# dbolya/yolact

Measured on AMD Instinct MI355X. Metric: images/sec (550x550, batch 8 per GPU), YOLACT yolact_resnet50 forward + Detect (Fast NMS), higher is better.
Workload: dtype f32 (fp32 in / fp32 accumulate / fp32 out; 92 % of the GEMM time on fp16x2 tiles = every fp32 operand as two fp16 pieces by round to nearest (22 significant bits + 2 signs: exact for ~2/3 of all fp32 values, one fp32 ulp otherwise), 3 exact piece products per product on the fp16 matrix pipe; measure

## Files before the change

yolact_amd/csrc/stem.hip:

```cpp
#include "common.h"
#include <stdlib.h>
#include "../../include/yolact_amd.h"

int ymi_internal_prof_begin(double flops, int tile, int kind, hipStream_t s);
void ymi_internal_prof_end(int idx, hipStream_t s);

namespace {

typedef _Float16 f16x8 __attribute__((ext_vector_type(8)));
typedef _Float16 f16x4 __attribute__((ext_vector_type(4)));

constexpr int NTHR = 512, NWAVE = 8;
constexpr int PH = 4, PW = 6;
constexpr int SH = 2 * PH + 1, SW = 2 * PW + 1;
constexpr int IH = 2 * SH + 5, IW = 2 * SW + 5;
constexpr int IPITCH = 32;
constexpr int NPATCH = IH * IPITCH;
constexpr int KPAD = 224, KSTEPS = KPAD / 16;
constexpr int WPITCH = KPAD * 2 + 16;
constexpr int COUT = 64;
constexpr int EPITCH = COUT + 1;

struct StemParams {
  const float *x; float *y;
  int B, H, W, Hs, Ws, Hp, Wp, tiles_x, tiles_y, ntiles;
  const unsigned short *w;
  int cout_pad;
  const float *scale, *bias;
  float *y_amax;
};

__device__ __forceinline__ int crow(int r, int lane) { return (r & 3) + 8 * (r >> 2) + 4 * (lane >> 5); }

__global__ __launch_bounds__(NTHR) void stem_pool_k(const StemParams p) {
#if defined(__HIP_DEVICE_COMPILE__)
  constexpr int WB = 0, WPLANE = COUT * WPITCH;
  constexpr int PB = 2 * WPLANE, PPLANE = NPATCH * 8;
  constexpr int EB = PB + 2 * PPLANE;
  constexpr int RED = EB + 128 * EPITCH * 4;
  constexpr int LDS_BYTES = RED + 64;
  static_assert(LDS_BYTES <= 160 * 1024, "LDS");
  __shared__ __attribute__((aligned(16))) unsigned char lds[LDS_BYTES];

  const int t = threadIdx.x, lane = t & 63, wave = __builtin_amdgcn_readfirstlane(t >> 6);
  const int hh = lane >> 5;
  const ymi_amax_pre apre = ymi_amax_prefetch(p.y_amax);

  for (int u = t; u < 2 * COUT * (KPAD / 8); u += NTHR) {
    const int plane = u / (COUT * (KPAD / 8)), r = u - plane * (COUT * (KPAD / 8));
    const int row = r / (KPAD / 8), g8 = r - row * (KPAD / 8);
    const f16x8 v = *reinterpret_cast<const f16x8 *>(p.w + ((size_t)plane * p.cout_pad + row) * KPAD + 8 * g8);
    *reinterpret_cast<f16x8 *>(lds + WB + plane * WPLANE + row * WPITCH + g8 * 16) = v;
  }
  const int mt = wave & 3, nt = wave >> 2;
  const int ncol = nt * 32 + (lane & 31);
  const float sc = p.scale[ncol], bi = p.bias[ncol];
  const int m = mt * 32 + (lane & 31);
  const int mi = m < SH * SW ? m / SW : 0, mj = m < SH * SW ? m - (m / SW) * SW : 0;
  const int abase = ((2 * mi) * IPITCH + 2 * mj) * 8;
  float *red = reinterpret_cast<float *>(lds + RED);
  float *et = reinterpret_cast<float *>(lds + EB);

  auto fetch = [&](int tile, float (&v)[2][3]) {
    const int b = tile / (p.tiles_x * p.tiles_y), tt = tile - b * (p.tiles_x * p.tiles_y);
    const int ty = tt / p.tiles_x, tx = tt - ty * p.tiles_x;
    const int iy0 = 4 * (ty * PH) - 5, ix0 = 4 * (tx * PW) - 5;
#pragma unroll
    for (int k = 0; k < 2; ++k) {
      const int slot = t + NTHR * k, r = slot >> 5, c = slot & 31;
      const int iy = iy0 + r, ix = ix0 + c;
      const bool ok = slot < NPATCH && c < IW && (unsigned)iy < (unsigned)p.H && (unsigned)ix < (unsigned)p.W;
      const float *src = p.x + ((size_t)b * 3 * p.H + (ok ? iy : 0)) * p.W + (ok ? ix : 0);
#pragma unroll
      for (int ch = 0; ch < 3; ++ch) v[k][ch] = ok ? src[(size_t)ch * p.H * p.W] : 0.f;
    }
  };
  float cur[2][3], nxt[2][3];
  int tile = blockIdx.x;
  if (tile < p.ntiles) fetch(tile, cur);
  float amy = 0.f;
  __syncthreads();
  for (; tile < p.ntiles; tile += gridDim.x) {
    const int b = tile / (p.tiles_x * p.tiles_y), tt = tile - b * (p.tiles_x * p.tiles_y);
    const int ty = tt / p.tiles_x, tx = tt - ty * p.tiles_x;
    float am = 0.f;
#pragma unroll
    for (int k = 0; k < 2; ++k)
#pragma unroll
      for (int ch = 0; ch < 3; ++ch) am = fmaxf(am, fabsf(cur[k][ch]));
    {
      const unsigned mx = ymi_wave_umax63(__float_as_uint(am));
      if (lane == 63) red[wave] = __uint_as_float(mx);
    }
    __syncthreads();
    float pm = 0.f;
#pragma unroll
    for (int w = 0; w < NWAVE; ++w) pm = fmaxf(pm, red[w]);
    float s, inv;
    ymi_h2_scale(pm, s, inv);
#pragma unroll
    for (int k = 0; k < 2; ++k) {
      const int slot = t + NTHR * k;
      if (slot < NPATCH) {
        f16x4 h, l;
#pragma unroll
        for (int ch = 0; ch < 3; ++ch) {
          const float tv = cur[k][ch] * s;
          h[ch] = (_Float16)tv;
          l[ch] = (_Float16)(tv - (float)h[ch]);
        }
        h[3] = (_Float16)0.f; l[3] = (_Float16)0.f;
        *reinterpret_cast<f16x4 *>(lds + PB + slot * 8) = h;
        *reinterpret_cast<f16x4 *>(lds + PB + PPLANE + slot * 8) = l;
      }
    }
    const int next = tile + gridDim.x;
    if (next < p.ntiles) fetch(next, nxt);
    __syncthreads();
    f32x16 acc;
#pragma unroll
    for (int r = 0; r < 16; ++r) acc[r] = 0.f;
    const unsigned char *wrow = lds + WB + ncol * WPITCH;
#pragma unroll
    for (int ks = 0; ks < KSTEPS; ++ks) {
      constexpr int NT = 49;
      const int ta0 = 4 * ks < NT ? 4 * ks : NT - 1, ta1 = 4 * ks + 1 < NT ? 4 * ks + 1 : NT - 1;
      const int tb0 = 4 * ks + 2 < NT ? 4 * ks + 2 : NT - 1, tb1 = 4 * ks + 3 < NT ? 4 * ks + 3 : NT - 1;
      const int oa0 = ((ta0 / 7) * IPITCH + ta0 % 7) * 8, oa1 = ((ta1 / 7) * IPITCH + ta1 % 7) * 8;
      const int ob0 = ((tb0 / 7) * IPITCH + tb0 % 7) * 8, ob1 = ((tb1 / 7) * IPITCH + tb1 % 7) * 8;
      const int o0 = abase + (hh ? ob0 : oa0), o1 = abase + (hh ? ob1 : oa1);
      const f16x4 h0 = *reinterpret_cast<const f16x4 *>(lds + PB + o0), h1 = *reinterpret_cast<const f16x4 *>(lds + PB + o1);
      const f16x4 l0 = *reinterpret_cast<const f16x4 *>(lds + PB + PPLANE + o0), l1 = *reinterpret_cast<const f16x4 *>(lds + PB + PPLANE + o1);
      const f16x8 ah = {h0[0], h0[1], h0[2], h0[3], h1[0], h1[1], h1[2], h1[3]};
      const f16x8 al = {l0[0], l0[1], l0[2], l0[3], l1[0], l1[1], l1[2], l1[3]};
      const f16x8 bh = *reinterpret_cast<const f16x8 *>(wrow + (16 * ks + 8 * hh) * 2);
      const f16x8 bl = *reinterpret_cast<const f16x8 *>(wrow + WPLANE + (16 * ks + 8 * hh) * 2);
      acc = ymi_mfma32(ah, bl, acc);
      acc = ymi_mfma32(al, bh, acc);
      acc = ymi_mfma32(ah, bh, acc);
    }
    const int sy0 = 2 * (ty * PH) - 1, sx0 = 2 * (tx * PW) - 1;
#pragma unroll
    for (int r = 0; r < 16; ++r) {
      const int row = mt * 32 + crow(r, lane);
      const int i = row / SW, j = row - i * SW;
      const bool ok = row < SH * SW && (unsigned)(sy0 + i) < (unsigned)p.Hs && (unsigned)(sx0 + j) < (unsigned)p.Ws;
      float v = (acc[r] * inv) * sc + bi;
      v = v > 0.f ? v : 0.f;
      et[row * EPITCH + ncol] = ok ? v : -__builtin_inff();
    }
    __syncthreads();
    const int c = t & 63;
#pragma unroll
    for (int k = 0; k < (PH * PW + 7) / 8; ++k) {
      const int q = (t >> 6) + 8 * k;
      if (q < PH * PW) {
        const int qy = q / PW, qx = q - qy * PW;
        const int py = ty * PH + qy, px = tx * PW + qx;
        float mx = -__builtin_inff();
#pragma unroll
        for (int dy = 0; dy < 3; ++dy)
#pragma unroll
          for (int dx = 0; dx < 3; ++dx) mx = fmaxf(mx, et[((2 * qy + dy) * SW + 2 * qx + dx) * EPITCH + c]);
        if (py < p.Hp && px < p.Wp) {
          p.y[(((size_t)b * p.Hp + py) * p.Wp + px) * COUT + c] = mx;
          amy = fmaxf(amy, fabsf(mx));
        }
      }
    }
#pragma unroll
    for (int k = 0; k < 2; ++k)
#pragma unroll
      for (int ch = 0; ch < 3; ++ch) cur[k][ch] = nxt[k][ch];
  }
  if (p.y_amax) ymi_amax_finish(apre, amy);
#endif
}

}

extern "C" int ymi_stem_pool_f32(const ymi_stem_desc *d, void *stream) {
  if (!d) return YMI_ENULL;
  if (!d->x || !d->y || !d->w_h2 || !d->scale_h2 || !d->bias) return YMI_ENULL;
  if (d->B <= 0 || d->H < 7 || d->W < 7) return YMI_EARG;
  if (d->cout_pad < COUT || d->kpad != KPAD) return YMI_ESHAPE;
  if ((((uintptr_t)d->w_h2) | ((uintptr_t)d->y)) & 15) return YMI_ESHAPE;
  StemParams p;
  p.x = d->x; p.y = d->y; p.B = d->B; p.H = d->H; p.W = d->W;
  p.Hs = (d->H + 6 - 7) / 2 + 1; p.Ws = (d->W + 6 - 7) / 2 + 1;
  p.Hp = (p.Hs + 2 - 3) / 2 + 1; p.Wp = (p.Ws + 2 - 3) / 2 + 1;
  if ((long)d->B * 3 * d->H * d->W >= (1L << 31) || (long)d->B * p.Hp * p.Wp * COUT >= (1L << 31)) return YMI_ESHAPE;
  p.tiles_x = (p.Wp + PW - 1) / PW; p.tiles_y = (p.Hp + PH - 1) / PH;
  p.ntiles = p.tiles_x * p.tiles_y * d->B;
  p.w = (const unsigned short *)d->w_h2; p.cout_pad = d->cout_pad;
  p.scale = d->scale_h2; p.bias = d->bias; p.y_amax = d->y_amax;
  hipStream_t s = (hipStream_t)stream;
  const double flops = 2.0 * d->B * p.Hs * p.Ws * 64.0 * 147.0;
  const int pr = ymi_internal_prof_begin(flops, YMI_TILE_H2 | YMI_TILE_64x64, 8, s);
  int dev = 0, cus = 256;
  hipGetDevice(&dev);
  hipDeviceGetAttribute(&cus, hipDeviceAttributeMultiprocessorCount, dev);
  const int grid = p.ntiles < cus ? p.ntiles : cus;
  hipLaunchKernelGGL(stem_pool_k, dim3(grid), dim3(NTHR), 0, s, p);
  const int rc = ymi_launch_status();
  ymi_internal_prof_end(pr, s);
  return rc;
}
```

Measured before the change: 2346.

## Restructure stem conv+pool kernel: smaller tiles, register weights, 2 WGs per CU

Shrinks the stem tile (3x4 pooled outputs, 64 M rows) and the workgroup to 256 threads so two workgroups fit per CU. The grid grows to twice the CU count. Weights move from LDS into registers, and the patch goes into a 4-phase parity layout to cut LDS bank conflicts. Interior tiles skip per-row bounds checks, and the pooling pass uses float4 loads and stores. The next-tile prefetch now overwrites the current register buffer, and optional timing stamps are gated behind YMI_DIAGNOSTICS. Smaller tiles increase halo redundancy and register pressure from keeping all weights resident.

```diff
diff --git a/yolact_amd/csrc/stem.hip b/yolact_amd/csrc/stem.hip
--- a/yolact_amd/csrc/stem.hip
+++ b/yolact_amd/csrc/stem.hip
@@ -10,16 +10,21 @@
 typedef _Float16 f16x8 __attribute__((ext_vector_type(8)));
 typedef _Float16 f16x4 __attribute__((ext_vector_type(4)));
 
-constexpr int NTHR = 512, NWAVE = 8;
-constexpr int PH = 4, PW = 6;
+constexpr int NTHR = 256, NWAVE = 4, WG_PER_CU = 2;
+constexpr int PH = 3, PW = 4;
 constexpr int SH = 2 * PH + 1, SW = 2 * PW + 1;
+constexpr int MROWS = 64;
 constexpr int IH = 2 * SH + 5, IW = 2 * SW + 5;
-constexpr int IPITCH = 32;
-constexpr int NPATCH = IH * IPITCH;
+constexpr int IPITCH = 24;
+constexpr int NFETCH = IH * IPITCH;
+constexpr int NF = (NFETCH + NTHR - 1) / NTHR;
+static_assert(SH * SW <= MROWS && IW <= IPITCH, "tile");
+constexpr int PPITCH = 41, PROWS = 11, PPLANE = PROWS * PPITCH;
+constexpr int NPSLOT = 4 * PPLANE;
+static_assert(PPITCH % 32 == SW % 32 && PPITCH >= (IW + 1) / 2 && PROWS >= (MROWS - 1) / SW + 4 && (NPSLOT * 8) % 16 == 0, "patch image");
 constexpr int KPAD = 224, KSTEPS = KPAD / 16;
-constexpr int WPITCH = KPAD * 2 + 16;
 constexpr int COUT = 64;
-constexpr int EPITCH = COUT + 1;
+constexpr int EPITCH = COUT;
 
 struct StemParams {
   const float *x; float *y;
@@ -28,80 +33,102 @@
   int cout_pad;
   const float *scale, *bias;
   float *y_amax;
+  unsigned long long *trace;
 };
 
+#ifdef YMI_DIAGNOSTICS
+#define STEM_STAMP(i) { const unsigned long long n_ = __builtin_amdgcn_s_memtime(); tr_[i] += n_ - last_; last_ = n_; }
+#else
+#define STEM_STAMP(i)
+#endif
+
+
 __device__ __forceinline__ int crow(int r, int lane) { return (r & 3) + 8 * (r >> 2) + 4 * (lane >> 5); }
-
-__global__ __launch_bounds__(NTHR) void stem_pool_k(const StemParams p) {
+__host__ __device__ constexpr int pslot(int r, int c) { return ((r & 1) * 2 + (c & 1)) * PPLANE + (r >> 1) * PPITCH + (c >> 1); }
+
+__global__ __launch_bounds__(NTHR, 2) void stem_pool_k(const StemParams p) {
 #if defined(__HIP_DEVICE_COMPILE__)
-  constexpr int WB = 0, WPLANE = COUT * WPITCH;
-  constexpr int PB = 2 * WPLANE, PPLANE = NPATCH * 8;
-  constexpr int EB = PB + 2 * PPLANE;
-  constexpr int RED = EB + 128 * EPITCH * 4;
-  constexpr int LDS_BYTES = RED + 64;
-  static_assert(LDS_BYTES <= 160 * 1024, "LDS");
+  constexpr int PB = 0, PL = NPSLOT * 8;
+  constexpr int EB = PB + 2 * PL;
+  constexpr int RED = EB + MROWS * EPITCH * 4;
+  constexpr int PIX = RED + 64;
+  constexpr int HALF = PIX + MROWS * 4;
+  constexpr int LDS_BYTES = HALF + NTHR * 4;
+  static_assert(WG_PER_CU * LDS_BYTES <= 160 * 1024, "LDS");
   __shared__ __attribute__((aligned(16))) unsigned char lds[LDS_BYTES];
 
   const int t = threadIdx.x, lane = t & 63, wave = __builtin_amdgcn_readfirstlane(t >> 6);
   const int hh = lane >> 5;
   const ymi_amax_pre apre = ymi_amax_prefetch(p.y_amax);
-
-  for (int u = t; u < 2 * COUT * (KPAD / 8); u += NTHR) {
-    const int plane = u / (COUT * (KPAD / 8)), r = u - plane * (COUT * (KPAD / 8));
-    const int row = r / (KPAD / 8), g8 = r - row * (KPAD / 8);
-    const f16x8 v = *reinterpret_cast<const f16x8 *>(p.w + ((size_t)plane * p.cout_pad + row) * KPAD + 8 * g8);
-    *reinterpret_cast<f16x8 *>(lds + WB + plane * WPLANE + row * WPITCH + g8 * 16) = v;
+#ifdef YMI_DIAGNOSTICS
+  unsigned long long tr_[8] = {0, 0, 0, 0, 0, 0, 0, 0}, last_ = __builtin_amdgcn_s_memtime();
+#endif
+
+  const int mw = wave & 1, nt = wave >> 1;
+  const int ncol = nt * 32 + (lane & 31);
+  f16x8 bh[KSTEPS], bl[KSTEPS];
+  {
+    const unsigned short *wr = p.w + (size_t)ncol * KPAD + 8 * hh;
+    const size_t plane = (size_t)p.cout_pad * KPAD;
+#pragma unroll
+    for (int ks = 0; ks < KSTEPS; ++ks) {
+      bh[ks] = *reinterpret_cast<const f16x8 *>(wr + 16 * ks);
+      bl[ks] = *reinterpret_cast<const f16x8 *>(wr + plane + 16 * ks);
+    }
   }
-  const int mt = wave & 3, nt = wave >> 2;
-  const int ncol = nt * 32 + (lane & 31);
+  for (int u = t; u < 2 * PL / 16; u += NTHR) *reinterpret_cast<f32x4 *>(lds + PB + u * 16) = f32x4{0.f, 0.f, 0.f, 0.f};
   const float sc = p.scale[ncol], bi = p.bias[ncol];
-  const int m = mt * 32 + (lane & 31);
-  const int mi = m < SH * SW ? m / SW : 0, mj = m < SH * SW ? m - (m / SW) * SW : 0;
-  const int abase = ((2 * mi) * IPITCH + 2 * mj) * 8;
+  const int m0 = mw * 32 + (lane & 31);
+  const int abase = ((m0 / SW) * PPITCH + m0 % SW) * 8;
   float *red = reinterpret_cast<float *>(lds + RED);
   float *et = reinterpret_cast<float *>(lds + EB);
-
-  auto fetch = [&](int tile, float (&v)[2][3]) {
+  int *pix = reinterpret_cast<int *>(lds + PIX);
+  if (t < MROWS) pix[t] = ((t / SW) << 8) | (t % SW);
+  reinterpret_cast<int *>(lds + HALF)[t] = hh;
+
+  auto fetch = [&](int tile, float (&v)[NF][3]) {
     const int b = tile / (p.tiles_x * p.tiles_y), tt = tile - b * (p.tiles_x * p.tiles_y);
     const int ty = tt / p.tiles_x, tx = tt - ty * p.tiles_x;
     const int iy0 = 4 * (ty * PH) - 5, ix0 = 4 * (tx * PW) - 5;
 #pragma unroll
-    for (int k = 0; k < 2; ++k) {
-      const int slot = t + NTHR * k, r = slot >> 5, c = slot & 31;
+    for (int k = 0; k < NF; ++k) {
+      const int slot = t + NTHR * k, r = slot / IPITCH, c = slot % IPITCH;
       const int iy = iy0 + r, ix = ix0 + c;
-      const bool ok = slot < NPATCH && c < IW && (unsigned)iy < (unsigned)p.H && (unsigned)ix < (unsigned)p.W;
+      const bool ok = slot < NFETCH && c < IW && (unsigned)iy < (unsigned)p.H && (unsigned)ix < (unsigned)p.W;
       const float *src = p.x + ((size_t)b * 3 * p.H + (ok ? iy : 0)) * p.W + (ok ? ix : 0);
 #pragma unroll
       for (int ch = 0; ch < 3; ++ch) v[k][ch] = ok ? src[(size_t)ch * p.H * p.W] : 0.f;
     }
   };
-  float cur[2][3], nxt[2][3];
+  float cur[NF][3];
   int tile = blockIdx.x;
   if (tile < p.ntiles) fetch(tile, cur);
   float amy = 0.f;
-  __syncthreads();
+  STEM_STAMP(0);
   for (; tile < p.ntiles; tile += gridDim.x) {
     const int b = tile / (p.tiles_x * p.tiles_y), tt = tile - b * (p.tiles_x * p.tiles_y);
     const int ty = tt / p.tiles_x, tx = tt - ty * p.tiles_x;
     float am = 0.f;
 #pragma unroll
-    for (int k = 0; k < 2; ++k)
+    for (int k = 0; k < NF; ++k)
 #pragma unroll
       for (int ch = 0; ch < 3; ++ch) am = fmaxf(am, fabsf(cur[k][ch]));
     {
       const unsigned mx = ymi_wave_umax63(__float_as_uint(am));
       if (lane == 63) red[wave] = __uint_as_float(mx);
     }
+    STEM_STAMP(1);
     __syncthreads();
+    STEM_STAMP(2);
     float pm = 0.f;
 #pragma unroll
     for (int w = 0; w < NWAVE; ++w) pm = fmaxf(pm, red[w]);
     float s, inv;
     ymi_h2_scale(pm, s, inv);
 #pragma unroll
-    for (int k = 0; k < 2; ++k) {
-      const int slot = t + NTHR * k;
-      if (slot < NPATCH) {
+    for (int k = 0; k < NF; ++k) {
+      const int slot = t + NTHR * k, r = slot / IPITCH, c = slot % IPITCH;
+      if (slot < NFETCH && c < IW) {
         f16x4 h, l;
 #pragma unroll
         for (int ch = 0; ch < 3; ++ch) {
@@ -110,70 +137,95 @@
           l[ch] = (_Float16)(tv - (float)h[ch]);
         }
         h[3] = (_Float16)0.f; l[3] = (_Float16)0.f;
-        *reinterpret_cast<f16x4 *>(lds + PB + slot * 8) = h;
-        *reinterpret_cast<f16x4 *>(lds + PB + PPLANE + slot * 8) = l;
+        *reinterpret_cast<f16x4 *>(lds + PB + pslot(r, c) * 8) = h;
+        *reinterpret_cast<f16x4 *>(lds + PB + PL + pslot(r, c) * 8) = l;
       }
     }
     const int next = tile + gridDim.x;
-    if (next < p.ntiles) fetch(next, nxt);
+    if (next < p.ntiles) fetch(next, cur);
+    STEM_STAMP(3);
     __syncthreads();
-    f32x16 acc;
-#pragma unroll
-    for (int r = 0; r < 16; ++r) acc[r] = 0.f;
-    const unsigned char *wrow = lds + WB + ncol * WPITCH;
-#pragma unroll
-    for (int ks = 0; ks < KSTEPS; ++ks) {
-      constexpr int NT = 49;
-      const int ta0 = 4 * ks < NT ? 4 * ks : NT - 1, ta1 = 4 * ks + 1 < NT ? 4 * ks + 1 : NT - 1;
-      const int tb0 = 4 * ks + 2 < NT ? 4 * ks + 2 : NT - 1, tb1 = 4 * ks + 3 < NT ? 4 * ks + 3 : NT - 1;
-      const int oa0 = ((ta0 / 7) * IPITCH + ta0 % 7) * 8, oa1 = ((ta1 / 7) * IPITCH + ta1 % 7) * 8;
-      const int ob0 = ((tb0 / 7) * IPITCH + tb0 % 7) * 8, ob1 = ((tb1 / 7) * IPITCH + tb1 % 7) * 8;
-      const int o0 = abase + (hh ? ob0 : oa0), o1 = abase + (hh ? ob1 : oa1);
-      const f16x4 h0 = *reinterpret_cast<const f16x4 *>(lds + PB + o0), h1 = *reinterpret_cast<const f16x4 *>(lds + PB + o1);
-      const f16x4 l0 = *reinterpret_cast<const f16x4 *>(lds + PB + PPLANE + o0), l1 = *reinterpret_cast<const f16x4 *>(lds + PB + PPLANE + o1);
-      const f16x8 ah = {h0[0], h0[1], h0[2], h0[3], h1[0], h1[1], h1[2], h1[3]};
-      const f16x8 al = {l0[0], l0[1], l0[2], l0[3], l1[0], l1[1], l1[2], l1[3]};
-      const f16x8 bh = *reinterpret_cast<const f16x8 *>(wrow + (16 * ks + 8 * hh) * 2);
-      const f16x8 bl = *reinterpret_cast<const f16x8 *>(wrow + WPLANE + (16 * ks + 8 * hh) * 2);
-      acc = ymi_mfma32(ah, bl, acc);
-      acc = ymi_mfma32(al, bh, acc);
-      acc = ymi_mfma32(ah, bh, acc);
-    }
+    STEM_STAMP(4);
+    const int hv = reinterpret_cast<const int *>(lds + HALF)[t];
     const int sy0 = 2 * (ty * PH) - 1, sx0 = 2 * (tx * PW) - 1;
-#pragma unroll
-    for (int r = 0; r < 16; ++r) {
-      const int row = mt * 32 + crow(r, lane);
-      const int i = row / SW, j = row - i * SW;
-      const bool ok = row < SH * SW && (unsigned)(sy0 + i) < (unsigned)p.Hs && (unsigned)(sx0 + j) < (unsigned)p.Ws;
-      float v = (acc[r] * inv) * sc + bi;
-      v = v > 0.f ? v : 0.f;
-      et[row * EPITCH + ncol] = ok ? v : -__builtin_inff();
-    }
+    const bool inner = sy0 >= 0 && sx0 >= 0 && sy0 + SH <= p.Hs && sx0 + SW <= p.Ws;
+    {
+      f32x16 acc;
+#pragma unroll
+      for (int r = 0; r < 16; ++r) acc[r] = 0.f;
+#pragma unroll
+      for (int ks = 0; ks < KSTEPS; ++ks) {
+        constexpr int NT = 49;
+        const int ta0 = 4 * ks < NT ? 4 * ks : NT - 1, ta1 = 4 * ks + 1 < NT ? 4 * ks + 1 : NT - 1;
+        const int tb0 = 4 * ks + 2 < NT ? 4 * ks + 2 : NT - 1, tb1 = 4 * ks + 3 < NT ? 4 * ks + 3 : NT - 1;
+        const int oa0 = pslot(ta0 / 7, ta0 % 7) * 8, oa1 = pslot(ta1 / 7, ta1 % 7) * 8;
+        const int ob0 = pslot(tb0 / 7, tb0 % 7) * 8, ob1 = pslot(tb1 / 7, tb1 % 7) * 8;
+        const unsigned char *q0 = lds + PB + abase + __mul24(hv, ob0 - oa0) + oa0;
+        const unsigned char *q1 = lds + PB + abase + __mul24(hv, ob1 - oa1) + oa1;
+        const f16x4 h0 = *reinterpret_cast<const f16x4 *>(q0), h1 = *reinterpret_cast<const f16x4 *>(q1);
+        const f16x4 l0 = *reinterpret_cast<const f16x4 *>(q0 + PL), l1 = *reinterpret_cast<const f16x4 *>(q1 + PL);
+        const f16x8 ah = {h0[0], h0[1], h0[2], h0[3], h1[0], h1[1], h1[2], h1[3]};
+        const f16x8 al = {l0[0], l0[1], l0[2], l0[3], l1[0], l1[1], l1[2], l1[3]};
+        acc = ymi_mfma32(ah, bl[ks], acc);
+        acc = ymi_mfma32(al, bh[ks], acc);
+        acc = ymi_mfma32(ah, bh[ks], acc);
+      }
+      float *erow = et + (mw * 32 + 4 * hh) * EPITCH + ncol;
+      if (inner) {
+#pragma unroll
+        for (int r = 0; r < 16; ++r) {
+          const float v = (acc[r] * inv) * sc + bi;
+          erow[crow(r, 0) * EPITCH] = v > 0.f ? v : 0.f;
+        }
+      } else {
+#pragma unroll
+        for (int r = 0; r < 16; ++r) {
+          const int ij = pix[mw * 32 + 4 * hh + crow(r, 0)];
+          const bool ok = (unsigned)(sy0 + (ij >> 8)) < (unsigned)p.Hs && (unsigned)(sx0 + (ij & 255)) < (unsigned)p.Ws;
+          float v = (acc[r] * inv) * sc + bi;
+          v = v > 0.f ? v : 0.f;
+          erow[crow(r, 0) * EPITCH] = ok ? v : -__builtin_inff();
+        }
+      }
+    }
+    STEM_STAMP(5);
     __syncthreads();
-    const int c = t & 63;
-#pragma unroll
-    for (int k = 0; k < (PH * PW + 7) / 8; ++k) {
-      const int q = (t >> 6) + 8 * k;
+    STEM_STAMP(6);
+    const int c4 = t & 15;
+#pragma unroll
+    for (int k = 0; k < (PH * PW * 16 + NTHR - 1) / NTHR; ++k) {
+      const int q = (t >> 4) + (NTHR / 16) * k;
       if (q < PH * PW) {
         const int qy = q / PW, qx = q - qy * PW;
         const int py = ty * PH + qy, px = tx * PW + qx;
-        float mx = -__builtin_inff();
-#pragma unroll
-        for (int dy = 0; dy < 3; ++dy)
-#pragma unroll
-          for (int dx = 0; dx < 3; ++dx) mx = fmaxf(mx, et[((2 * qy + dy) * SW + 2 * qx + dx) * EPITCH + c]);
+        f32x4 mx;
+#pragma unroll
+        for (int dx = 0; dx < 3; ++dx) {
+          const float *e = et + ((2 * qy) * SW + 2 * qx + dx) * EPITCH + 4 * c4;
+          const f32x4 v0 = *reinterpret_cast<const f32x4 *>(e), v1 = *reinterpret_cast<const f32x4 *>(e + SW * EPITCH);
+          const f32x4 v2 = *reinterpret_cast<const f32x4 *>(e + 2 * SW * EPITCH);
+#pragma unroll
+          for (int ch = 0; ch < 4; ++ch) {
+            const float cm = fmaxf(fmaxf(v0[ch], v1[ch]), v2[ch]);
+            mx[ch] = dx ? fmaxf(mx[ch], cm) : cm;
+          }
+        }
         if (py < p.Hp && px < p.Wp) {
-          p.y[(((size_t)b * p.Hp + py) * p.Wp + px) * COUT + c] = mx;
-          amy = fmaxf(amy, fabsf(mx));
-        }
-      }
-    }
-#pragma unroll
-    for (int k = 0; k < 2; ++k)
-#pragma unroll
-      for (int ch = 0; ch < 3; ++ch) cur[k][ch] = nxt[k][ch];
+          *reinterpret_cast<f32x4 *>(p.y + (((size_t)b * p.Hp + py) * p.Wp + px) * COUT + 4 * c4) = mx;
+          amy = fmaxf(amy, ymi_absmax4(mx));
+        }
+      }
+    }
+    STEM_STAMP(7);
   }
   if (p.y_amax) ymi_amax_finish(apre, amy);
+#ifdef YMI_DIAGNOSTICS
+  if (p.trace && lane == 0 && (wave == 0 || wave == 3)) {
+    unsigned long long *o_ = p.trace + 16 * (size_t)blockIdx.x + (wave == 0 ? 0 : 8);
+#pragma unroll
+    for (int i = 0; i < 8; ++i) o_[i] = tr_[i];
+  }
+#endif
 #endif
 }
 
@@ -194,13 +246,20 @@
   p.ntiles = p.tiles_x * p.tiles_y * d->B;
   p.w = (const unsigned short *)d->w_h2; p.cout_pad = d->cout_pad;
   p.scale = d->scale_h2; p.bias = d->bias; p.y_amax = d->y_amax;
+  p.trace = nullptr;
+#ifdef YMI_DIAGNOSTICS
+  { const char *e = getenv("YMI_STEM_TRACE"); p.trace = e ? (unsigned long long *)strtoull(e, nullptr, 0) : nullptr; }
+#endif
   hipStream_t s = (hipStream_t)stream;
   const double flops = 2.0 * d->B * p.Hs * p.Ws * 64.0 * 147.0;
   const int pr = ymi_internal_prof_begin(flops, YMI_TILE_H2 | YMI_TILE_64x64, 8, s);
   int dev = 0, cus = 256;
   hipGetDevice(&dev);
   hipDeviceGetAttribute(&cus, hipDeviceAttributeMultiprocessorCount, dev);
-  const int grid = p.ntiles < cus ? p.ntiles : cus;
+  int grid = p.ntiles < WG_PER_CU * cus ? p.ntiles : WG_PER_CU * cus;
+#ifdef YMI_DIAGNOSTICS
+  { const char *e = getenv("YMI_STEM_GRID"); if (e && atoi(e) > 0 && atoi(e) < grid) grid = atoi(e); }
+#endif
   hipLaunchKernelGGL(stem_pool_k, dim3(grid), dim3(NTHR), 0, s, p);
   const int rc = ymi_launch_status();
   ymi_internal_prof_end(pr, s);
```

New measurement: 2359, median of 3. Within noise of the previous version (+0.6%).
